# Gepeng18/Sentinel

Hardware: AMD Instinct MI355X
Metric: admission decisions/sec at 1M rules Zipf(1.1), 1/2/4/8 GPU; % HBM peak (higher is better)
Workload: dtype int64

## Files before the change

sentinel_amd/csrc/cluster.hip:

```cpp
#include "cluster.hpp"
#include "cluster_exact.hpp"
#include "cparam_exact.hpp"

#include <cstdio>
#include <cstdlib>

#include <algorithm>
#include <type_traits>

namespace sga {

namespace {

constexpr int kThreads = 256;
constexpr int kItems = 16;
constexpr int kTileElems = kThreads * kItems;

enum : uint8_t { RUN_FAST = 0, RUN_DONE = 1 };

__device__ __forceinline__ uint64_t lanemask_lt64(int lane) { return (1ULL << lane) - 1ULL; }

__device__ __forceinline__ HashEntry slot_lookup(const ClusterState &st, int64_t fid) {
    uint32_t h = (uint32_t)hash_flow_id(fid) & st.hmask;
    for (uint32_t probe = 0; probe <= st.hmask; ++probe) {
// ... 1876 lines not shown
            sc.seg_stat[kSegStat * seg] = a;
        }
        __syncthreads();
        if (active) {
            uint32_t npc = 0;
            for (int w = 0; w < wave; ++w) npc += s_np[w];
            const uint32_t pgper = (((n + kHotSeg - 1) / kHotSeg) + kPsGroups - 1) / kPsGroups;
#pragma unroll
            for (int r = 0; r < kSubRounds; ++r) {
                const uint32_t i = ubase + (uint32_t)r * 64 + lane;
                const uint32_t cd = hc[r];
                const bool hot = i < send && cd != kNoCode;
                const uint32_t hid = cd & 0xFFFu;
                const uint32_t r_seg = hot ? ((cd >> 12) & 0x1FFFu) + c[hid] : 0u;
                const bool pr = hot && (cd >> 31);
                if (i < send) sc.hcode[i] = hot ? ((cd & ~(0x1FFFu << 12)) | (r_seg << 12)) : kNoCode;
                const uint64_t em = __ballot(pr);
                if (pr) {
                    sc.pel_tile[(size_t)seg * kHotSeg + npc + (uint32_t)__popcll(em & lt)] = el_pack(hid, r_seg >> 7, 1u, r_seg & 127u, i);
                    atomicAdd(&sc.prow[(size_t)(seg / pgper) * kHot + hid], 1u);
                }
                npc += (uint32_t)__popcll(em);
            }
        }
        __syncthreads();
        const uint32_t b0 = sh.s_bmin, b1 = sh.s_bmax;
        uint32_t *pc = reinterpret_cast<uint32_t *>(&cnt[0][0]);
        for (uint32_t b = b0; b <= b1; ++b) {
            for (uint32_t k = threadIdx.x; k < nhot; k += kKeyThreads) pc[k] = 0;
            __syncthreads();
#pragma unroll
            for (int r = 0; r < kSubRounds; ++r) {
                const uint32_t cd = hc[r];
                if (ubase + (uint32_t)r * 64 + lane < send && cd != kNoCode && ((cd >> 25) & 63u) < b)
                    atomicAdd(&pc[cd & 0xFFFu], 1u);
            }
            __syncthreads();
            for (uint32_t k = threadIdx.x; k < nhot; k += kKeyThreads) sc.hpre[(size_t)b * kHot + k] = (uint16_t)pc[k];
            if (threadIdx.x == 0) atomicAdd(&sc.counters[CTL_NPRE], 1u);
            __syncthreads();
        }
    }
    {
        tmax_l = wave_max_u32(tmax_l);
        if (lane == 0) {
            sh.s_tm[wave] = tmax_l;
            sh.s_nc[wave] = nc;
        }
        __syncthreads();
        if (threadIdx.x == 0) {
            uint32_t tm = 0, a = 0, p = 0, bd = 0;
            for (int w = 0; w < kKeyWaves; ++w) {
                tm = max(tm, sh.s_tm[w]);
                a += sh.s_nc[w];
                if (nhot) {
                    p += s_np[w];
                    bd = max(bd, s_bd[w]);
                }
            }
            if (kPass == 0) {
                uint32_t *kt = sc.ktot + (seg % kKeyStripes) * kKeyStripeWords;
                if (a) atomicAdd(&kt[0], a);
                if (p) atomicAdd(&kt[1], p);
                if (bd) atomicMax(&kt[2], bd);
                if (tm) atomicMax(&kt[3], tm);
            } else if (a) {
                atomicAdd(&sc.counters[CTL_NSORT], a);
            }
        }
    }
    if (lane == 0) sc.tile_nc[sub] = active ? nc : 0u;
    if (pl) {
        __syncthreads();
        for (uint32_t k = threadIdx.x; k < (uint32_t)kPartBins; k += kKeyThreads)
            hist[(size_t)seg * kPartBins + k] = sh.phist[k];
    }
    if (d0) {
        __syncthreads();
        for (uint32_t k = threadIdx.x; k < (2u << d0); k += kKeyThreads) {
            const uint32_t t = k >> d0, d = k & dmask, tile = seg * 2 + t;
            if (tile < ntiles) hist[(size_t)d * ntiles + tile] = sh.hist0[t][d];
        }
    }
}

__global__ __launch_bounds__(256) void k_part_colscan(BatchScratch sc, uint32_t nseg) {
    const uint32_t b = blockIdx.x * 256 + threadIdx.x;
    const uint32_t t0 = blockIdx.y * kPartGroup, t1 = min(nseg, t0 + kPartGroup);
    uint32_t acc = 0;
    for (uint32_t t = t0; t < t1; t += 8) {
        uint32_t v[8];
#pragma unroll
        for (int k = 0; k < 8; ++k) v[k] = t + k < t1 ? sc.phist[(size_t)(t + k) * kPartBins + b] : 0u;
#pragma unroll
        for (int k = 0; k < 8; ++k) {
            if (t + k < t1) sc.phist[(size_t)(t + k) * kPartBins + b] = acc;
            acc += v[k];
        }
    }
    sc.pgrp[(size_t)blockIdx.y * kPartBins + b] = acc;
}

__global__ __launch_bounds__(256) void k_part_binscan(BatchScratch sc, uint32_t ngroups) {
    __shared__ uint32_t ws[4];
    __shared__ uint32_t s_last;
    const int lane = threadIdx.x & 63, wave = threadIdx.x >> 6;
    const uint32_t b = blockIdx.x * 256 + threadIdx.x;
    uint32_t acc = 0;
    for (uint32_t g = 0; g < ngroups; g += 8) {
        uint32_t v[8];
#pragma unroll
        for (int k = 0; k < 8; ++k) v[k] = g + k < ngroups ? sc.pgrp[(size_t)(g + k) * kPartBins + b] : 0u;
#pragma unroll
        for (int k = 0; k < 8; ++k) {
            if (g + k < ngroups) sc.pgrp[(size_t)(g + k) * kPartBins + b] = acc;
            acc += v[k];
        }
    }
    sc.pstart[b] = acc;
    __threadfence();
    __syncthreads();
    if (threadIdx.x == 0) s_last = atomicAdd(&sc.pstart[kPartBins + 1], 1u) == gridDim.x - 1;
    __syncthreads();
    if (!s_last) return;
    __threadfence();
    constexpr int kPer = kPartBins / 256;
    uint32_t tot[kPer], ts = 0;
#pragma unroll
    for (int k = 0; k < kPer; ++k) {
        tot[k] = __hip_atomic_load(&sc.pstart[threadIdx.x * kPer + k], __ATOMIC_RELAXED, __HIP_MEMORY_SCOPE_AGENT);
        ts += tot[k];
    }
    uint32_t x = ts;
#pragma unroll
    for (int o = 1; o < 64; o <<= 1) {
        const uint32_t y = __shfl_up(x, o, 64);
        if (lane >= o) x += y;
    }
    if (lane == 63) ws[wave] = x;
    __syncthreads();
    uint32_t pre = x - ts;
    for (int w = 0; w < wave; ++w) pre += ws[w];
#pragma unroll
    for (int k = 0; k < kPer; ++k) {
        sc.pstart[threadIdx.x * kPer + k] = pre;
        pre += tot[k];
    }
    if (threadIdx.x == 255) {
        sc.pstart[kPartBins] = pre;
        sc.pstart[kPartBins + 1] = 0;
    }
}

__global__ __launch_bounds__(kKeyThreads) void k_part_scatter(BatchScratch sc, uint32_t nseg, int lb,
                                                              uint64_t *__restrict__ out) {
    __shared__ uint32_t gb[kPartBins];
    __shared__ uint16_t wc[kKeyWaves][kPartBins];
    const uint32_t per = (nseg + 7) / 8;
    const uint32_t seg = (blockIdx.x & 7u) * per + (blockIdx.x >> 3);
    if (seg >= nseg) return;
    const uint32_t g = seg / kPartGroup;
    const int lane = threadIdx.x & 63, wave = threadIdx.x >> 6;
    const uint64_t lt = lanemask_lt64(lane);
    for (uint32_t b = threadIdx.x; b < (uint32_t)kPartBins; b += kKeyThreads) {
        gb[b] = sc.pstart[b] + sc.pgrp[(size_t)g * kPartBins + b] + sc.phist[(size_t)seg * kPartBins + b];
#pragma unroll
        for (int w = 0; w < kKeyWaves; ++w) wc[w][b] = 0;
    }
    const uint32_t sub = seg * kKeyWaves + wave;
    const uint32_t nc = sc.tile_nc[sub];
    const uint64_t *src = sc.el_tile + (size_t)sub * kSubSeg;
    uint64_t x[kSubRounds];
#pragma unroll
    for (int r = 0; r < kSubRounds; ++r) {
        const uint32_t i = (uint32_t)r * 64 + lane;
        x[r] = src[i < nc ? i : 0u];
    }
    __syncthreads();
#pragma unroll
    for (int r = 0; r < kSubRounds; ++r) {
        if ((uint32_t)r * 64 >= nc) break;
        const bool valid = (uint32_t)r * 64 + lane < nc;
        const uint32_t b = el_slot(x[r]) >> lb;
        const uint64_t peers = match_lanes(b, kPartBits, valid);
        if (valid && (peers & lt) == 0) wc[wave][b] += (uint16_t)__popcll(peers);
        __builtin_amdgcn_wave_barrier();
    }
    __syncthreads();
    for (uint32_t b = threadIdx.x; b < (uint32_t)kPartBins; b += kKeyThreads) {
        uint32_t run = 0;
#pragma unroll
        for (int w = 0; w < kKeyWaves; ++w) {
            const uint32_t c = wc[w][b];
            wc[w][b] = (uint16_t)run;
            run += c;
        }
    }
    __syncthreads();
#pragma unroll
    for (int r = 0; r < kSubRounds; ++r) {
        if ((uint32_t)r * 64 >= nc) break;
        const bool valid = (uint32_t)r * 64 + lane < nc;
        const uint32_t b = el_slot(x[r]) >> lb;
        const uint64_t peers = match_lanes(b, kPartBits, valid);
        if (valid) out[gb[b] + wc[wave][b] + (uint32_t)__popcll(peers & lt)] = x[r];
        __builtin_amdgcn_wave_barrier();
        if (valid && (peers & lt) == 0) wc[wave][b] += (uint16_t)__popcll(peers);
        __builtin_amdgcn_wave_barrier();
    }
}

template <int kPass, bool kDense, bool kNT, bool kPk>
__device__ __forceinline__ void hot_key_pass(KeyShared &sh, const ClusterState &st, const BatchScratch &sc,
                                             const ReqIn &in, int64_t ts_base, uint32_t n, uint64_t *__restrict__ out,
                                             int d0, uint32_t *__restrict__ hist, uint32_t ntiles, int pipelined) {
    const uint32_t nseg = (n + kHotSeg - 1) / kHotSeg;
    if (kPass == 0) {
        if (blockIdx.x >= nseg) {
            const uint32_t fl = hot_precheck(st, sc, in, ts_base, (blockIdx.x - nseg) * kKeyThreads + threadIdx.x,
                                             pipelined);
            if (fl) atomicOr(&sc.counters[CTL_FLAGS], fl);
            return;
        }
        hot_key<0, kDense, kNT, kPk>(sh, st, sc, in, ts_base, n, out, d0, hist, ntiles, blockIdx.x);
        return;
    }
    const uint32_t f = sc.counters[CTL_FLAGS];
    const bool rerun = (f & (kFlagRerun | kFlagState)) != 0;
    if (blockIdx.x == 0 && threadIdx.x < (uint32_t)kKeyStripes) {
        static_assert(kKeyStripes == 64, "one stripe per lane of the first wave");
        uint32_t *kt = sc.ktot + threadIdx.x * kKeyStripeWords;
        uint32_t ns = kt[0], np = kt[1], bd = kt[2], tm = kt[3];
        kt[0] = kt[1] = kt[2] = kt[3] = 0;
        ns = wave_sum_u32(ns);
        np = wave_sum_u32(np);
        bd = wave_max_u32(bd);
        tm = wave_max_u32(tm);
        if (threadIdx.x == 0) {
            atomicMax(sc.tmax_all, (unsigned long long)(ts_base + (int64_t)tm));
            if (!rerun) {
                sc.counters[CTL_NSORT] = ns;
                sc.counters[CTL_NPRIO] = np;
                sc.counters[CTL_NCOLD] = ns;
                sc.counters[CTL_BDHI] = bd;
                sc.counters[CTL_MODE] = hot_count(sc) ? 1u : 0u;
            }
        }
    }
    if (!rerun) return;
    for (uint32_t seg = blockIdx.x; seg < nseg; seg += gridDim.x) {
        hot_key<1, kDense, kNT, kPk>(sh, st, sc, in, ts_base, n, out, d0, hist, ntiles, seg);
        __syncthreads();
    }
    __threadfence();
    __syncthreads();
    if (threadIdx.x == 0) sh.s_last = atomicAdd(&sc.counters[CTL_KTICKET], 1u) == gridDim.x - 1;
    __syncthreads();
    if (!sh.s_last || threadIdx.x != 0) return;
    __threadfence();
    const uint32_t ns = ld_agent(&sc.counters[CTL_NSORT]);
    sc.counters[CTL_NCOLD] = ns;
    sc.counters[CTL_NPRIO] = 0;
    sc.counters[CTL_BDHI] = 0;
    sc.counters[CTL_MODE] = 0;
    sc.counters[CTL_KTICKET] = 0;
    if (f & kFlagState) {
        sc.counters[CTL_FLAGS] = kFlagState;
        sc.counters[CTL_BDLO] = 0;
        sc.counters[CTL_NPRE] = 0;
    }
}

template <int kPass, bool kNT = false, bool kPk = false>
__global__ __launch_bounds__(kKeyThreads) __attribute__((amdgpu_waves_per_eu(4))) void k_hot_key_dense(
    ClusterState st, BatchScratch sc, ReqIn in, int64_t ts_base, uint32_t n, uint64_t *__restrict__ out, int d0,
    uint32_t *__restrict__ hist, uint32_t ntiles, int pipelined) {
    __shared__ KeyShared sh;
    hot_key_pass<kPass, true, kNT, kPk>(sh, st, sc, in, ts_base, n, out, d0, hist, ntiles, pipelined);
}
template <int kPass, bool kPk = false>
__global__ __launch_bounds__(kKeyThreads) void k_hot_key_hash(
    ClusterState st, BatchScratch sc, ReqIn in, int64_t ts_base, uint32_t n, uint64_t *__restrict__ out, int d0,
    uint32_t *__restrict__ hist, uint32_t ntiles, int pipelined) {
    __shared__ KeyShared sh;
    hot_key_pass<kPass, false, false, kPk>(sh, st, sc, in, ts_base, n, out, d0, hist, ntiles, pipelined);
}

__global__ __launch_bounds__(kThreads) void k_hscan_group(BatchScratch sc, uint32_t nrows) {
    if (!sc.counters[CTL_MODE]) return;
    const uint32_t h = blockIdx.y * kThreads + threadIdx.x;
    if (h >= hot_count(sc)) return;
    const uint32_t r0 = blockIdx.x * kHotGroupRows;
    uint32_t s = 0;
#pragma unroll
    for (int k = 0; k < kHotGroupRows; ++k)
        if (r0 + k < nrows) s += sc.hcnt[(size_t)(r0 + k) * kHot + h];
    sc.hgsum[(size_t)blockIdx.x * kHot + h] = s;
}

__device__ __forceinline__ void psort_cols_one(const BatchScratch &sc, uint32_t h, uint32_t ngroups);
__global__ __launch_bounds__(kThreads) void k_hscan_mid(BatchScratch sc, uint32_t ngroups, uint32_t pgroups) {
    if (!sc.counters[CTL_MODE]) return;
    const uint32_t h = blockIdx.x * kThreads + threadIdx.x;
    if (pgroups) psort_cols_one(sc, h, pgroups);
    if (h >= hot_count(sc)) return;
    uint32_t acc = 0;
#pragma unroll 8
    for (uint32_t g = 0; g < ngroups; ++g) {
        const uint32_t v = sc.hgsum[(size_t)g * kHot + h];
        sc.hgsum[(size_t)g * kHot + h] = acc;
        acc += v;
    }
    sc.hot_tot[h] = acc;
}

__global__ __launch_bounds__(kThreads) void k_hscan_down(BatchScratch sc, uint32_t nrows) {
    if (!sc.counters[CTL_MODE]) return;
    const uint32_t h = blockIdx.y * kThreads + threadIdx.x;
    if (h >= hot_count(sc)) return;
    const uint32_t r0 = blockIdx.x * kHotGroupRows;
    uint32_t v[kHotGroupRows];
#pragma unroll
    for (int k = 0; k < kHotGroupRows; ++k) v[k] = r0 + k < nrows ? sc.hcnt[(size_t)(r0 + k) * kHot + h] : 0u;
    uint32_t run = sc.hgsum[(size_t)blockIdx.x * kHot + h];
#pragma unroll
    for (int k = 0; k < kHotGroupRows; ++k) {
        if (r0 + k < nrows) sc.hbase[(size_t)(r0 + k) * kHot + h] = run;
        run += v[k];
    }
}

__device__ __forceinline__ uint32_t ps_per_group(uint32_t nseg) { return (nseg + kPsGroups - 1) / kPsGroups; }

__global__ __launch_bounds__(256) void k_psort_cols(BatchScratch sc, uint32_t ngroups) {
    if (!sc.counters[CTL_MODE]) return;
    psort_cols_one(sc, blockIdx.x * 256 + threadIdx.x, ngroups);
}
__device__ __forceinline__ void psort_cols_one(const BatchScratch &sc, uint32_t h, uint32_t ngroups) {
    uint32_t acc = 0;
    constexpr int kChunk = 64;
    for (uint32_t g0 = 0; g0 < ngroups; g0 += kChunk) {
        uint32_t v[kChunk];
#pragma unroll
        for (int k = 0; k < kChunk; ++k) v[k] = g0 + k < ngroups ? sc.prow[(size_t)(g0 + k) * kHot + h] : 0u;
#pragma unroll
        for (int k = 0; k < kChunk; ++k) {
            if (g0 + k < ngroups) sc.ppre[(size_t)(g0 + k) * kHot + h] = acc;
            acc += v[k];
        }
    }
    sc.ptot[h] = acc;
}

__global__ __launch_bounds__(64) void k_psort_scatter(BatchScratch sc, uint32_t nseg, uint64_t *__restrict__ out) {
    __shared__ uint32_t base[kHot];
    const uint32_t g = blockIdx.x;
    const int lane = threadIdx.x;
    const bool mode = sc.counters[CTL_MODE] != 0;
    if (mode) {
        constexpr int kPer = kHot / 64;
        uint32_t sum = 0;
// ... 1266 lines not shown
    take(sc.phist, segs_alloc * kPartBins * 4);
    take(sc.pgrp, ((segs_alloc + kPartGroup - 1) / kPartGroup) * kPartBins * 4);
    take(sc.pstart, (kPartBins + 2) * 4);
    return off;
}

size_t batch_scratch_bytes(size_t cap, uint32_t nslots_cap) {
    BatchScratch none;
    return batch_scratch_layout(none, nullptr, cap, nslots_cap);
}

void batch_scratch_carve(BatchScratch &sc, void *base, size_t cap, uint32_t nslots_cap) {
    batch_scratch_layout(sc, (char *)base, cap, nslots_cap);
    sc.counters_clean = 0;
    sc.cap = cap;
    SGA_HIP_CHECK(hipMemset(sc.prow, 0, (size_t)kPsGroups * kHot * 4));
    SGA_HIP_CHECK(hipMemset(sc.ktot, 0, kKeyStripes * kKeyStripeWords * 4));
}

__device__ __forceinline__ uint32_t probe_mix(uint32_t x) {
    x ^= x >> 16;
    x *= 0x7feb352dU;
    x ^= x >> 15;
    x *= 0x846ca68bU;
    x ^= x >> 16;
    return x;
}
__global__ __launch_bounds__(kThreads) void k_lds_order_probe(uint32_t *bad) {
    __shared__ uint32_t cw[kThreads / 64][kHot / 2];
    const int lane = threadIdx.x & 63, w = threadIdx.x >> 6;
    const uint32_t K = 1u << (blockIdx.x % 13);
    const int mode = (blockIdx.x / 13) % 3;
    for (int k = lane; k < kHot / 2; k += 64) cw[w][k] = 0;
    __builtin_amdgcn_wave_barrier();
    const uint64_t lt = lanemask_lt64(lane);
    uint32_t nb = 0;
    for (uint32_t r = 0; r < 32; ++r) {
        const uint32_t x = probe_mix((blockIdx.x * 1315423911u) ^ (r * 2654435761u) ^ (threadIdx.x * 97u));
        uint32_t hid = x % K;
        if (mode == 1 && (x & 1u)) hid = 7 % K;
        const bool act = mode == 2 ? ((x >> 8) & 1u) : true;
        const uint32_t sh = (hid & 1u) << 4;
        const uint32_t before = (cw[w][hid >> 1] >> sh) & 0xFFFFu;
        __builtin_amdgcn_wave_barrier();
        uint64_t peers = __ballot(act);
        for (int b = 0; b < 12; ++b) {
            const bool bit = (hid >> b) & 1u;
            const uint64_t bb = __ballot(bit);
            peers &= bit ? bb : ~bb;
        }
        const uint32_t expect = before + (uint32_t)__popcll(peers & lt);
        __builtin_amdgcn_wave_barrier();
        uint32_t got = expect;
        if (act) got = rank_hot(cw[w], hid);
        __builtin_amdgcn_wave_barrier();
        if (got != expect) ++nb;
    }
    if (nb) atomicAdd(bad, nb);
}

bool lds_lane_order_ok(hipStream_t s) {
    uint32_t *d = nullptr, h = 1;
    if (hipMalloc(&d, 4) != hipSuccess) return false;
    bool ok = hipMemsetAsync(d, 0, 4, s) == hipSuccess;
    if (ok) {
        hipLaunchKernelGGL(k_lds_order_probe, dim3(13 * 3 * 64), dim3(kThreads), 0, s, d);
        ok = hipMemcpyAsync(&h, d, 4, hipMemcpyDeviceToHost, s) == hipSuccess &&
             hipStreamSynchronize(s) == hipSuccess && h == 0;
    }
    (void)hipFree(d);
    return ok;
}

void hot_reset(const ClusterState &st, BatchScratch &sc, uint32_t nslots_cap, hipStream_t s) {
    const uint32_t m = std::max(nslots_cap, st.dkey ? st.dense_n : 0u);
    hipLaunchKernelGGL(k_hot_reset, dim3(std::max<uint32_t>(1, std::min<uint32_t>((m + 255) / 256, 4096))),
                       dim3(256), 0, s, st, sc, nslots_cap);
}

static void side_stream_init(BatchScratch &sc) {
    if (sc.side) return;
    SGA_HIP_CHECK(hipStreamCreateWithFlags(&sc.side, hipStreamNonBlocking));
    const unsigned evf = hipEventDisableTiming | hipEventReleaseToDevice;
    SGA_HIP_CHECK(hipEventCreateWithFlags(&sc.ev_fork0, evf));
    SGA_HIP_CHECK(hipEventCreateWithFlags(&sc.ev_fork, evf));
    SGA_HIP_CHECK(hipEventCreateWithFlags(&sc.ev_join, evf));
    SGA_HIP_CHECK(hipEventCreateWithFlags(&sc.ev_mid, evf));
    SGA_HIP_CHECK(hipStreamCreateWithFlags(&sc.side2, hipStreamNonBlocking));
    SGA_HIP_CHECK(hipEventCreateWithFlags(&sc.ev_prio, evf));
}

static int cold_part_lb(int bits) {
    const int lb = bits - kPartBits;
    return (lb >= 5 && lb <= kPartMaxLow) ? lb : 0;
}

static int hot_key_bits(const ClusterState &st) {
    int bits = 1;
    while (((uint64_t)1 << bits) < (uint64_t)st.nslots + kHot + 2) ++bits;
    return bits;
}

static int hot_key_d0(const BatchScratch &sc, int bits) {
    const int dsort = radix64_digit_bits(bits);
    return sc.part_lb ? -sc.part_lb : (dsort <= 8 ? dsort : 0);
}

static uint32_t hot_nseg(uint32_t n) { return (n + kHotSeg - 1) / kHotSeg; }

static void hot_key_passes(const ClusterState &st, BatchScratch &sc, const ReqIn &in, int64_t ts_base, uint32_t n,
                           uint64_t *out, hipStream_t s, bool clean, bool pipelined) {
    const int bits = hot_key_bits(st);
    const uint32_t nseg = hot_nseg(n);
    if (!clean) {
        SGA_HIP_CHECK(hipMemsetAsync(sc.counters, 0, CTL_WORDS * 4, s));
        SGA_HIP_CHECK(hipMemsetAsync(sc.ktot, 0, kKeyStripes * kKeyStripeWords * 4, s));
    }
    const bool pk = in.pk != nullptr;
    auto hka = st.dense_n ? (pk ? k_hot_key_dense<0, true, true> : k_hot_key_dense<0, true, false>)
                          : (pk ? k_hot_key_hash<0, true> : k_hot_key_hash<0, false>);
    auto hkb = st.dense_n ? (pk ? k_hot_key_dense<1, false, true> : k_hot_key_dense<1, false, false>)
                          : (pk ? k_hot_key_hash<1, true> : k_hot_key_hash<1, false>);
    sc.part_lb = cold_part_lb(bits);
    const int d0 = hot_key_d0(sc, bits);
    const uint32_t ntiles_sort = (uint32_t)radix64_tiles(n);
    uint32_t *khist = sc.part_lb ? sc.phist : sc.radix.hist;
    hipLaunchKernelGGL(hka, dim3(nseg + kPreWgs), dim3(kKeyThreads), 0, s, st, sc, in, ts_base, n, out, d0, khist,
                       ntiles_sort, pipelined ? 1 : 0);
    hipLaunchKernelGGL(hkb, dim3(std::min<uint32_t>(nseg, 256)), dim3(kKeyThreads), 0, s, st, sc, in, ts_base, n, out,
                       d0, khist, ntiles_sort, 0);
}

static uint32_t ps_per_group_h(uint32_t nseg) { return std::max<uint32_t>(1, (nseg + kPsGroups - 1) / kPsGroups); }
static uint32_t ps_groups_h(uint32_t nseg) { return (nseg + ps_per_group_h(nseg) - 1) / ps_per_group_h(nseg); }

static void hot_scans(BatchScratch &sc, uint32_t nseg, uint32_t pgroups, hipStream_t hs) {
    const uint32_t ngroups = (nseg + kHotGroupRows - 1) / kHotGroupRows;
    hipLaunchKernelGGL(k_hscan_group, dim3(ngroups, kHot / kThreads), dim3(kThreads), 0, hs, sc, nseg);
    hipLaunchKernelGGL(k_hscan_mid, dim3(kHot / kThreads), dim3(kThreads), 0, hs, sc, ngroups, pgroups);
    hipLaunchKernelGGL(k_hscan_down, dim3(ngroups, kHot / kThreads), dim3(kThreads), 0, hs, sc, nseg);
}

static void prio_scatter(BatchScratch &sc, uint32_t nseg, hipStream_t ps) {
    hipLaunchKernelGGL(k_psort_scatter, dim3(kPsGroups), dim3(64), 0, ps, sc, nseg, sc.pel[0]);
    sc.pel_sorted = sc.pel[0];
}

static void cold_order(const ClusterState &st, BatchScratch &sc, uint32_t n, hipStream_t s) {
    const uint32_t nseg = hot_nseg(n);
    if (sc.part_lb) {
        const uint32_t ngroups = (nseg + kPartGroup - 1) / kPartGroup;
        hipLaunchKernelGGL(k_part_colscan, dim3(kPartBins / 256, ngroups), dim3(256), 0, s, sc, nseg);
        hipLaunchKernelGGL(k_part_binscan, dim3(kPartBins / 256), dim3(256), 0, s, sc, ngroups);
        hipLaunchKernelGGL(k_part_scatter, dim3(8 * ((nseg + 7) / 8)), dim3(kKeyThreads), 0, s, sc, nseg, sc.part_lb,
                           sc.el[0]);
        sc.el_sorted = sc.el[0];
    } else {
        const int bits = hot_key_bits(st);
        const int np = radix_sort_u64_tiled(sc.el_tile, sc.tile_nc, sc.counters + CTL_NSORT, sc.el[0], sc.el[1], n,
                                            kSlotShift, bits, sc.radix, s, hot_key_d0(sc, bits) > 0);
        sc.el_sorted = (np & 1) ? sc.el[0] : sc.el[1];
    }
}

static void hot_side(const ClusterState &st, BatchScratch &sc, int64_t ts_base, uint32_t n, uint64_t *out,
                     hipStream_t hs) {
    const uint32_t pgrid = std::max<uint32_t>(1, std::min<uint32_t>((n + kThreads - 1) / kThreads, 1024));
    hipLaunchKernelGGL(k_prio_rank, dim3(pgrid), dim3(kThreads), 0, hs, st, sc, sc.pel_sorted);
    hipLaunchKernelGGL(k_hot_flows, dim3(kHot / kH1Waves), dim3(kThreads), 0, hs, st, sc, ts_base);
    SGA_HIP_CHECK(hipEventRecord(sc.ev_mid, hs));
    hipLaunchKernelGGL(k_hot_final_g, dim3((n + kFinGSpan - 1) / kFinGSpan + kFinPrioWgsG), dim3(kFinGThreads), 0, hs,
                       st, sc, n, sc.pel_sorted, out);
    SGA_HIP_CHECK(hipEventRecord(sc.ev_join, hs));
}

static void cold_stage_and_next(const ClusterState &st, BatchScratch &sc, const ReqIn &in, int64_t ts_base,
                                uint32_t n, uint64_t *out, hipStream_t s) {
    const uint32_t hot_min = std::max<uint32_t>(sc.hot_min, 1);
    cold_stage(st, sc, sc.el_sorted, n, sc.counters + CTL_NCOLD, st.nslots, in, ts_base, 0, hot_min, out, s,
               sc.part_lb);
    if (fz_debug()) {
        unsigned long long ph[8];
        SGA_HIP_CHECK(hipMemcpyFromSymbolAsync(ph, HIP_SYMBOL(g_fz_phase), sizeof(ph), 0, hipMemcpyDeviceToHost, s));
        SGA_HIP_CHECK(hipStreamSynchronize(s));
        const unsigned long long z[8] = {0, 0, 0, 0, 0, 0, 0, 0};
        SGA_HIP_CHECK(hipMemcpyToSymbolAsync(HIP_SYMBOL(g_fz_phase), z, sizeof(z), 0, hipMemcpyHostToDevice, s));
        if (ph[7])
            fprintf(stderr, "fz phases (wall_clock64 ticks per workgroup, %llu wgs): order %.0f runs %.0f flows %.0f results %.0f\n",
                    ph[7], (double)ph[3] / ph[7], (double)ph[0] / ph[7], (double)ph[1] / ph[7], (double)ph[2] / ph[7]);
    }
    SGA_HIP_CHECK(hipStreamWaitEvent(s, sc.ev_mid, 0));
    const uint32_t sb = 64;
    hipLaunchKernelGGL(k_hot_next_a, dim3(sb), dim3(kThreads), 0, s, st, sc, hot_min);
    hipLaunchKernelGGL(k_hot_pick, dim3(sb), dim3(kThreads), 0, s, st, sc, sc.hot_min);
    SGA_HIP_CHECK(hipStreamWaitEvent(s, sc.ev_join, 0));
    hipLaunchKernelGGL(k_hot_fin, dim3(1), dim3(kFinThreads), 0, s, st, sc);
    sc.counters_clean = 1;
}

static void decide_hot_sync(const ClusterState &st, BatchScratch &sc, const ReqIn &in, int64_t ts_base, uint32_t n,
                            uint64_t *out, hipStream_t s, bool clean) {
    const uint32_t nseg = hot_nseg(n);
    hot_key_passes(st, sc, in, ts_base, n, out, s, clean, false);
    side_stream_init(sc);
    SGA_HIP_CHECK(hipEventRecord(sc.ev_fork0, s));
    SGA_HIP_CHECK(hipStreamWaitEvent(sc.side, sc.ev_fork0, 0));
    hot_scans(sc, nseg, ps_groups_h(nseg), sc.side);
    prio_scatter(sc, nseg, sc.side);
    hot_side(st, sc, ts_base, n, out, sc.side);
    cold_order(st, sc, n, s);
    cold_stage_and_next(st, sc, in, ts_base, n, out, s);
}

bool cluster_hot_eligible(const ClusterState &st, const BatchScratch &sc, uint32_t n, int simple, int nlims) {
    const bool limited = nlims > 0 && !simple;
    if (n == 0 || (n <= std::min<uint32_t>(sc.small_max, kSmall) && !limited && !radix64_lookback())) return false;
    return sc.hot_enabled && sc.hot_lane_order && !simple && !limited && !radix64_lookback() &&
           st.nslots + (uint64_t)kHot + 2 < kMaxSlots;
}

void cluster_classify_hot(const ClusterState &st, BatchScratch &sc, const int64_t *flow_id, const int32_t *acquire,
                          const uint8_t *prio, int64_t ts_base, const uint32_t *ts_off, uint32_t n, void *out,
                          hipStream_t s) {
    const bool clean = sc.counters_clean != 0;
    sc.counters_clean = 0;
    test_dispatch_reset(s);
    ReqIn in;
    in.flow = flow_id;
    in.acq = acquire;
    in.prio = prio;
    in.ts = ts_off;
    const uint32_t nseg = hot_nseg(n);
    hot_key_passes(st, sc, in, ts_base, n, (uint64_t *)out, s, clean, true);
    side_stream_init(sc);
    SGA_HIP_CHECK(hipEventRecord(sc.ev_fork0, s));
    SGA_HIP_CHECK(hipStreamWaitEvent(sc.side, sc.ev_fork0, 0));
    SGA_HIP_CHECK(hipStreamWaitEvent(sc.side2, sc.ev_fork0, 0));
    hot_scans(sc, nseg, 0u, sc.side);
    hipLaunchKernelGGL(k_psort_cols, dim3(kHot / 256), dim3(256), 0, sc.side2, sc, ps_groups_h(nseg));
    prio_scatter(sc, nseg, sc.side2);
    SGA_HIP_CHECK(hipEventRecord(sc.ev_prio, sc.side2));
    SGA_HIP_CHECK(hipStreamWaitEvent(sc.side, sc.ev_prio, 0));
    cold_order(st, sc, n, s);
    SGA_HIP_CHECK(hipEventRecord(sc.ev_fork, sc.side));
    SGA_HIP_CHECK(hipStreamWaitEvent(s, sc.ev_fork, 0));
}

void cluster_decide_hot(const ClusterState &st, BatchScratch &sc, const int32_t *acquire, const uint8_t *prio,
                        int64_t ts_base, const uint32_t *ts_off, uint32_t n, void *out, hipStream_t s) {
    ReqIn in;
    in.acq = acquire;
    in.prio = prio;
    in.ts = ts_off;
    SGA_HIP_CHECK(hipEventRecord(sc.ev_fork0, s));
    SGA_HIP_CHECK(hipStreamWaitEvent(sc.side, sc.ev_fork0, 0));
    hot_side(st, sc, ts_base, n, (uint64_t *)out, sc.side);
    cold_stage_and_next(st, sc, in, ts_base, n, (uint64_t *)out, s);
}

void cluster_decide_batch(const ClusterState &st, BatchScratch &sc, const int64_t *flow_id, const int32_t *acquire,
                          const uint8_t *prio, int64_t ts_base, const uint32_t *ts_off, uint32_t n, int simple,
                          void *out_v, hipStream_t s, const LimiterPass *lims, int nlims) {
    if (n == 0) return;
    test_dispatch_reset(s);
    ReqIn in;
    in.flow = flow_id;
    in.acq = acquire;
    in.prio = simple ? nullptr : prio;
    in.ts = ts_off;
    const bool clean = sc.counters_clean != 0;
    sc.counters_clean = 0;
    uint64_t *out = (uint64_t *)out_v;
    int bits = 1;
    while (((uint64_t)1 << bits) < (uint64_t)st.nslots + 1) ++bits;
    const uint32_t invalid_key = st.nslots;
    const bool limited = nlims > 0 && !simple;
    const int d0 = radix64_digit_bits(bits);
    const uint32_t ntiles = (n + kTileElems - 1) / kTileElems;
    static_assert(kTileElems == kRadix64Tile, "classify tiles are sort tiles");
    const bool lb = radix64_lookback() != 0;
    const int npass = (bits + d0 - 1) / d0;
    if (lb && (npass << d0) > 1024)
        throw HipError("look-back sort (SGA_RADIX_MODE=0) needs npass << digit bits <= 1024", __FILE__, __LINE__);
    if (n <= std::min<uint32_t>(sc.small_max, kSmall) && !limited && !lb) {
        uint32_t m = 64;
        while (m < n) m <<= 1;
        hipLaunchKernelGGL(k_small_sort, dim3(1), dim3(kSmallThreads), 0, s, st, flow_id, acquire, prio, ts_off, ts_base,
                           n, m, simple, invalid_key, sc.el[0], out);
        hipLaunchKernelGGL(k_cold_fused, dim3((n + kFzChunk - 1) / kFzChunk), dim3(kFzThreads), 0, s, st, sc, sc.el[0],
                           n, nullptr, invalid_key, in, ts_base, simple, 0xFFFFFFFFu, out, 0, nullptr, 0);
        return;
    }
    if (cluster_hot_eligible(st, sc, n, simple, nlims)) {
        decide_hot_sync(st, sc, in, ts_base, n, out, s, clean);
        return;
    }
    SGA_HIP_CHECK(hipMemsetAsync(sc.counters, 0, CTL_WORDS * 4, s));
    if (lb) SGA_HIP_CHECK(hipMemsetAsync(sc.radix.ghist, 0, kRadixGhistWords * sizeof(uint32_t), s));
    if (lb) SGA_HIP_CHECK(hipMemsetAsync(sc.radix.err, 0, sizeof(uint32_t), s));
    const uint64_t *el = sc.el[npass & 1];
    hipLaunchKernelGGL(k_classify, dim3(ntiles), dim3(kThreads), 0, s, st, flow_id, acquire, prio, ts_off, ts_base, n,
                       simple, invalid_key, sc.el[0], out, limited ? 0 : d0, ntiles, sc.radix.hist,
                       (lb && !limited) ? npass : 0, bits, sc.radix.ghist);
    if (!simple) apply_limiters(st.param, sc, sc.el[0], n, invalid_key, ts_base, ts_off, out, lims, nlims, s);
    const int np = radix_sort_u64(sc.el[0], sc.el[1], n, kSlotShift, bits, sc.radix, s, !limited);
    if (np != npass) throw HipError("radix pass count mismatch", __FILE__, __LINE__);
    cold_stage(st, sc, el, n, nullptr, invalid_key, in, ts_base, simple, 0xFFFFFFFFu, out, s, 0);
// ... 272 lines not shown
```

sentinel_amd/csrc/cluster.hpp:

```cpp
#pragma once
#include "../../include/sentinel_amd.h"
#include "common.hpp"
#include "radix_sort.hpp"

namespace sga {

struct SlotParam {
    double thr;
    double thr_simple;
    double isec;
    uint32_t boff;
    int32_t S;
    int32_t W;
    int32_t interval;
    int32_t active;
    int32_t ns;
};

struct SlotOcc {
    int64_t occ_pass;
    int64_t occ_preq;
    int32_t has_occ;
    int32_t pad;
};

enum : int { CEV_PASS = 0, CEV_BLOCK, CEV_PASS_REQUEST, CEV_BLOCK_REQUEST, CEV_OCCUPIED_PASS, CEV_OCCUPIED_BLOCK,
             CEV_WAITING, CEV_N };

struct alignas(16) HashEntry {
    int64_t key;
    uint32_t slot;
    uint32_t W;
};

struct ClusterState {
    const SlotParam *param;
    int64_t *rec;
    const HashEntry *htab;
    const uint32_t *dense;
    uint32_t *dkey;
    const uint32_t *wtab;
    const int64_t *slot_fid;
    uint32_t dense_n;
    uint32_t hmask;
    uint32_t nslots;
    double max_occupy_ratio;
    int32_t uni_S, uni_W, uni_iv, uni_pad;
};

constexpr uint32_t kDkHot = 0x80000000u, kDkNone = 0x7FFFFFFFu;

struct ReqIn {
    const int64_t *flow = nullptr;
    const int32_t *acq = nullptr;
    const uint8_t *prio = nullptr;
    const uint32_t *ts = nullptr;
    const uint32_t *pk = nullptr;
    __device__ __forceinline__ uint32_t ts_at(uint32_t i) const { return pk ? pk[3 * (size_t)i + 1] : ts[i]; }
    __device__ __forceinline__ int32_t acq_at(uint32_t i) const {
        return pk ? (int32_t)(pk[3 * (size_t)i + 2] & 0xFFFFu) : acq[i];
    }
    __device__ __forceinline__ bool prio_at(uint32_t i) const {
        return pk ? ((pk[3 * (size_t)i + 2] >> 16) & 1u) != 0 : (prio && prio[i]);
    }
    __device__ __forceinline__ int64_t flow_at(uint32_t i) const { return pk ? (int64_t)pk[3 * (size_t)i] : flow[i]; }
};

struct NsLimiterDev {
    int64_t start[10];
    int64_t cnt[10];
};

struct LimiterPass {
    int32_t ns;
    double qps_allowed;
    NsLimiterDev *state;
};

struct alignas(16) RunOut {
    int64_t s0;
    double thr;
    double isec;
    uint32_t f;
    uint32_t cpf;
    uint32_t cw;
    uint16_t wait;
    uint8_t mode;
    uint8_t pad;
};

struct RAgg {
    uint32_t nh, flag, cnt;
};

struct HotRun {
    int64_t s0;
    double thr;
    double isec;
    uint32_t f;
    uint32_t start;
    uint32_t n;
    uint32_t p0;
    uint32_t cpf;
    uint32_t cw;
    uint16_t wait;
    uint8_t ok;
    uint8_t pad;
    uint32_t pad2[3];
};
static_assert(sizeof(HotRun) == 64, "hot run record");

constexpr int kHot = 4096;
constexpr uint16_t kColdId = 0xFFFF;
constexpr uint32_t kNoSlot = 0xFFFFFFFFu;
constexpr int kHotCtlWords = 128;
constexpr int kHotSeg = 8192;
constexpr int kSubSeg = 1024;
constexpr int kHotBuckets = 64;
constexpr int kHotGroupRows = 16;
constexpr int kHotCand = 1 << 16;
constexpr int kSegStat = 4;
constexpr int kKeyStripes = 64;
constexpr int kKeyStripeWords = 32;
constexpr int kPartBits = 11;
constexpr int kPartBins = 1 << kPartBits;
constexpr int kPartGroup = 64;
constexpr int kPartMaxLow = 10;

enum : int {
    CTL_NVALID = 0, CTL_NRUNS = 1, CTL_NFLOWS = 2, CTL_LIMITED = 4, CTL_LIMRUNS = 5, CTL_DEFERRED = 6,
    CTL_FLAGS = 16,
    CTL_NPRIO = 19,
    CTL_NSORT = 20,
    CTL_NCOLD = 21,
    CTL_NPRE = 22,
    CTL_BDLO = 23,
    CTL_BDHI = 24,
    CTL_MODE = 25,
    CTL_HOTERR = 26,
    CTL_KTICKET = 27,
    CTL_WORDS = 64
};
enum : uint32_t {
    kFlagUnsorted = 1,
    kFlagMixed = 2,
    kFlagBucket = 4,
    kFlagHotKey = 8,
    kFlagRerun = 15,
    kFlagState = 16
};

struct WConst {
    uint32_t W, r0;
    double inv;
};

struct BatchScratch {
    uint64_t *el[2];
    uint32_t *run_start, *run_slot, *run_idx0, *run_cp, *run_p0;
    int32_t *run_acq;
    uint8_t *run_bd;
    uint32_t *flow_first_run;
    uint32_t *plist;
    RunOut *run_out;
    RAgg *wave_carry;
    void *tile_agg;
    void *tile_carry;
    uint32_t *tile_valid;
    uint32_t *counters;
    uint32_t *counters_last;
    int counters_clean = 0;
    uint32_t *lim_partial;
    RadixScratch radix;
    size_t cap = 0;
    uint16_t *hot_of;
    uint32_t *hot_slot;
    uint32_t *hot_next;
    uint32_t *hot_ctl;
    uint64_t *el_tile;
    uint32_t *tile_nc;
    uint64_t *pel_tile;
    uint32_t *prow;
    uint32_t *ppre;
    uint32_t *ptot;
    uint64_t *pel[2];
    uint32_t *hcode;
    uint16_t *hcnt;
    uint32_t *hbase;
    uint32_t *hgsum;
    uint16_t *hpre;
    uint32_t *hbnd;
    HotRun *hrun;
    uint32_t *prank;
    uint32_t *plo, *phi;
    uint32_t *hot_tot;
    uint32_t *seg_stat;
    uint32_t *ktot;
    unsigned long long *tmax_all;
    const uint64_t *el_sorted = nullptr, *pel_sorted = nullptr;
    uint32_t *hot_cand;
    uint32_t *phist, *pgrp, *pstart;
    int part_lb = 0;
    int hot_enabled = 1;
    uint32_t small_max = 4096;
    int hot_lane_order = 0;
    uint32_t hot_min = 64;
    hipStream_t side = nullptr;
    hipEvent_t ev_fork = nullptr, ev_join = nullptr, ev_fork0 = nullptr, ev_mid = nullptr;
    hipStream_t side2 = nullptr;
    hipEvent_t ev_prio = nullptr;
};

bool lds_lane_order_ok(hipStream_t stream);

void hot_reset(const ClusterState &st, BatchScratch &b, uint32_t nslots_cap, hipStream_t stream);
void batch_scratch_release(BatchScratch &b);

constexpr size_t kMaxBatch = (size_t)1 << 26;
constexpr uint32_t kMaxSlots = (1u << 24) - 2;

size_t batch_scratch_bytes(size_t cap, uint32_t nslots_cap);
void batch_scratch_carve(BatchScratch &b, void *base, size_t cap, uint32_t nslots_cap);

void cluster_decide_batch(const ClusterState &st, BatchScratch &sc, const int64_t *flow_id, const int32_t *acquire,
                          const uint8_t *prio, int64_t ts_base, const uint32_t *ts_off, uint32_t n, int simple,
                          void *out , hipStream_t stream, const LimiterPass *lims = nullptr,
                          int nlims = 0);
void cluster_decide_batch_packed(const ClusterState &st, BatchScratch &sc, const uint32_t *pk, int64_t ts_base,
                                 uint32_t n, void *out, hipStream_t stream, const LimiterPass *lims = nullptr,
                                 int nlims = 0);

bool cluster_hot_eligible(const ClusterState &st, const BatchScratch &sc, uint32_t n, int simple, int nlims);
void cluster_classify_hot(const ClusterState &st, BatchScratch &sc, const int64_t *flow_id, const int32_t *acquire,
                          const uint8_t *prio, int64_t ts_base, const uint32_t *ts_off, uint32_t n, void *out,
                          hipStream_t stream);
void cluster_decide_hot(const ClusterState &st, BatchScratch &sc, const int32_t *acquire, const uint8_t *prio,
                        int64_t ts_base, const uint32_t *ts_off, uint32_t n, void *out, hipStream_t stream);

struct PRuleParam {
    double count;
    double isec;
    uint32_t boff;
    int32_t S, W, interval;
    int32_t active, ns, threshold_type;
    uint32_t hot_off, n_hot;
    uint32_t cap;
};

struct PLruRec {
    uint64_t kidx;
    uint64_t stamp;
};
constexpr uint64_t kPNoQueue = ~0ull;
constexpr uint64_t kPLruBuilding = ~0ull;

struct CParamState {
    const PRuleParam *param;
    int64_t *rstart;
    int64_t *tmax;
    uint8_t *coupled;
    const HashEntry *htab;
    uint32_t hmask, nslots;
    const int64_t *hot_v;
    const int32_t *hot_c;
    const int32_t *ns_connected;
    int64_t *vtab;
    uint32_t vmask;
    uint64_t *ktab;
    uint32_t kmask;
    uint32_t *koff;
    uint32_t *kslot;
    int64_t *kval;
    int64_t *krec;
    uint64_t krec_cap;
    uint32_t *ctl;
    uint32_t *nkeys;
    uint64_t *pq;
    uint32_t *psize;
    PLruRec *lpool;
// ... 46 lines not shown
```

Measured before the change: 24.43 billion.

## Scatter two partition segments per workgroup with atomic counting and vectorized bin init

```diff
diff --git a/sentinel_amd/csrc/cluster.hip b/sentinel_amd/csrc/cluster.hip
--- a/sentinel_amd/csrc/cluster.hip
+++ b/sentinel_amd/csrc/cluster.hip
@@ -2052,39 +2052,92 @@
     }
 }
 
+__device__ __forceinline__ void part_list(const BatchScratch &sc, uint32_t sub0, uint32_t nsub, int lane,
+                                          uint32_t (&cum)[kPartSpan + 1]) {
+    const uint32_t mine = lane < kPartSpan && sub0 + (uint32_t)lane < nsub ? sc.tile_nc[sub0 + lane] : 0u;
+    cum[0] = 0;
+#pragma unroll
+    for (int j = 0; j < kPartSpan; ++j) cum[j + 1] = cum[j] + (uint32_t)__builtin_amdgcn_readlane((int)mine, j);
+}
+
+__device__ __forceinline__ void part_load(const BatchScratch &sc, uint32_t sub0, const uint32_t (&cum)[kPartSpan + 1],
+                                          uint32_t c0, int lane, uint64_t (&x)[kSubRounds]) {
+#pragma unroll
+    for (int r = 0; r < kSubRounds; ++r) {
+        const uint32_t i = c0 + (uint32_t)r * 64 + lane;
+        uint32_t at = i;
+#pragma unroll
+        for (int j = 1; j < kPartSpan; ++j)
+            if (i >= cum[j]) at = (uint32_t)j * kSubSeg + (i - cum[j]);
+        x[r] = i < cum[kPartSpan] ? sc.el_tile[(size_t)sub0 * kSubSeg + at] : 0ull;
+    }
+}
+
+__device__ __forceinline__ void part_count_add(uint16_t *wcw, uint32_t b) {
+    (void)__hip_atomic_fetch_add(reinterpret_cast<uint32_t *>(wcw) + (b >> 1), 1u << ((b & 1u) * 16), __ATOMIC_RELAXED,
+                                 __HIP_MEMORY_SCOPE_WORKGROUP);
+}
+__device__ __forceinline__ void part_count_add(uint32_t *wcw, uint32_t b) {
+    (void)__hip_atomic_fetch_add(wcw + b, 1u, __ATOMIC_RELAXED, __HIP_MEMORY_SCOPE_WORKGROUP);
+}
+
+template <bool kPlace, typename Cnt>
+__device__ __forceinline__ void part_rounds(const uint64_t (&x)[kSubRounds], uint32_t c0, uint32_t total,
+                                            const uint32_t *gb, Cnt *wcw, int lb, uint64_t *__restrict__ out,
+                                            int lane) {
+    const uint64_t lt = lanemask_lt64(lane);
+#pragma unroll
+    for (int r = 0; r < kSubRounds; ++r) {
+        if (c0 + (uint32_t)r * 64 >= total) break;
+        const bool valid = c0 + (uint32_t)r * 64 + lane < total;
+        const uint32_t b = el_slot(x[r]) >> lb;
+        if (!kPlace) {
+            if (valid) part_count_add(wcw, b);
+            continue;
+        }
+        const uint64_t peers = match_lanes(b, kPartBits, valid);
+        if (valid) out[gb[b] + wcw[b] + (uint32_t)__popcll(peers & lt)] = x[r];
+        __builtin_amdgcn_wave_barrier();
+        if (valid && (peers & lt) == 0) wcw[b] += (Cnt)__popcll(peers);
+        __builtin_amdgcn_wave_barrier();
+    }
+}
+
 __global__ __launch_bounds__(kKeyThreads) void k_part_scatter(BatchScratch sc, uint32_t nseg, int lb,
                                                               uint64_t *__restrict__ out) {
-    __shared__ uint32_t gb[kPartBins];
-    __shared__ uint16_t wc[kKeyWaves][kPartBins];
-    const uint32_t per = (nseg + 7) / 8;
-    const uint32_t seg = (blockIdx.x & 7u) * per + (blockIdx.x >> 3);
-    if (seg >= nseg) return;
-    const uint32_t g = seg / kPartGroup;
+    static_assert(kPartBins == 4 * kKeyThreads, "four consecutive bins per thread");
+    using Cnt = std::conditional_t<(kPartSpan * kHotSeg <= 65535), uint16_t, uint32_t>;
+    __shared__ __attribute__((aligned(16))) uint32_t gb[kPartBins];
+    __shared__ __attribute__((aligned(16))) Cnt wc[kKeyWaves][kPartBins];
+    const uint32_t nspan = (nseg + kPartSpan - 1) / kPartSpan;
+    const uint32_t per = (nspan + 7) / 8;
+    const uint32_t span = (blockIdx.x & 7u) * per + (blockIdx.x >> 3);
+    if (span >= nspan) return;
+    const uint32_t seg0 = span * kPartSpan;
+    const uint32_t g = seg0 / kPartGroup;
     const int lane = threadIdx.x & 63, wave = threadIdx.x >> 6;
-    const uint64_t lt = lanemask_lt64(lane);
-    for (uint32_t b = threadIdx.x; b < (uint32_t)kPartBins; b += kKeyThreads) {
-        gb[b] = sc.pstart[b] + sc.pgrp[(size_t)g * kPartBins + b] + sc.phist[(size_t)seg * kPartBins + b];
-#pragma unroll
-        for (int w = 0; w < kKeyWaves; ++w) wc[w][b] = 0;
-    }
-    const uint32_t sub = seg * kKeyWaves + wave;
-    const uint32_t nc = sc.tile_nc[sub];
-    const uint64_t *src = sc.el_tile + (size_t)sub * kSubSeg;
+    const uint32_t sub0 = seg0 * kKeyWaves + (uint32_t)wave * kPartSpan;
+    uint32_t cum[kPartSpan + 1];
+    part_list(sc, sub0, nseg * kKeyWaves, lane, cum);
+    const uint32_t total = cum[kPartSpan];
     uint64_t x[kSubRounds];
-#pragma unroll
-    for (int r = 0; r < kSubRounds; ++r) {
-        const uint32_t i = (uint32_t)r * 64 + lane;
-        x[r] = src[i < nc ? i : 0u];
+    part_load(sc, sub0, cum, 0u, lane, x);
+    const uint32_t b4 = threadIdx.x * 4;
+    const uint4 st4 = *reinterpret_cast<const uint4 *>(sc.pstart + b4);
+    const uint4 gp = *reinterpret_cast<const uint4 *>(sc.pgrp + (size_t)g * kPartBins + b4);
+    const uint4 row = *reinterpret_cast<const uint4 *>(sc.phist + (size_t)seg0 * kPartBins + b4);
+    *reinterpret_cast<uint4 *>(&gb[b4]) =
+        make_uint4(st4.x + gp.x + row.x, st4.y + gp.y + row.y, st4.z + gp.z + row.z, st4.w + gp.w + row.w);
+    {
+        uint32_t *z = reinterpret_cast<uint32_t *>(&wc[0][0]);
+        for (uint32_t i = threadIdx.x; i < (uint32_t)(sizeof(wc) / 4); i += kKeyThreads) z[i] = 0;
     }
     __syncthreads();
-#pragma unroll
-    for (int r = 0; r < kSubRounds; ++r) {
-        if ((uint32_t)r * 64 >= nc) break;
-        const bool valid = (uint32_t)r * 64 + lane < nc;
-        const uint32_t b = el_slot(x[r]) >> lb;
-        const uint64_t peers = match_lanes(b, kPartBits, valid);
-        if (valid && (peers & lt) == 0) wc[wave][b] += (uint16_t)__popcll(peers);
-        __builtin_amdgcn_wave_barrier();
+    for (uint32_t c0 = 0;;) {
+        part_rounds<false>(x, c0, total, gb, wc[wave], lb, out, lane);
+        c0 += kSubSeg;
+        if (c0 >= total) break;
+        part_load(sc, sub0, cum, c0, lane, x);
     }
     __syncthreads();
     for (uint32_t b = threadIdx.x; b < (uint32_t)kPartBins; b += kKeyThreads) {
@@ -2092,21 +2145,14 @@
 #pragma unroll
         for (int w = 0; w < kKeyWaves; ++w) {
             const uint32_t c = wc[w][b];
-            wc[w][b] = (uint16_t)run;
+            wc[w][b] = (Cnt)run;
             run += c;
         }
     }
     __syncthreads();
-#pragma unroll
-    for (int r = 0; r < kSubRounds; ++r) {
-        if ((uint32_t)r * 64 >= nc) break;
-        const bool valid = (uint32_t)r * 64 + lane < nc;
-        const uint32_t b = el_slot(x[r]) >> lb;
-        const uint64_t peers = match_lanes(b, kPartBits, valid);
-        if (valid) out[gb[b] + wc[wave][b] + (uint32_t)__popcll(peers & lt)] = x[r];
-        __builtin_amdgcn_wave_barrier();
-        if (valid && (peers & lt) == 0) wc[wave][b] += (uint16_t)__popcll(peers);
-        __builtin_amdgcn_wave_barrier();
+    for (uint32_t c0 = 0; c0 < total; c0 += kSubSeg) {
+        if (total > (uint32_t)kSubSeg) part_load(sc, sub0, cum, c0, lane, x);
+        part_rounds<true>(x, c0, total, gb, wc[wave], lb, out, lane);
     }
 }
 
@@ -3679,7 +3725,8 @@
         const uint32_t ngroups = (nseg + kPartGroup - 1) / kPartGroup;
         hipLaunchKernelGGL(k_part_colscan, dim3(kPartBins / 256, ngroups), dim3(256), 0, s, sc, nseg);
         hipLaunchKernelGGL(k_part_binscan, dim3(kPartBins / 256), dim3(256), 0, s, sc, ngroups);
-        hipLaunchKernelGGL(k_part_scatter, dim3(8 * ((nseg + 7) / 8)), dim3(kKeyThreads), 0, s, sc, nseg, sc.part_lb,
+        const uint32_t nspan = (nseg + kPartSpan - 1) / kPartSpan;
+        hipLaunchKernelGGL(k_part_scatter, dim3(8 * ((nspan + 7) / 8)), dim3(kKeyThreads), 0, s, sc, nseg, sc.part_lb,
                            sc.el[0]);
         sc.el_sorted = sc.el[0];
     } else {
diff --git a/sentinel_amd/csrc/cluster.hpp b/sentinel_amd/csrc/cluster.hpp
--- a/sentinel_amd/csrc/cluster.hpp
+++ b/sentinel_amd/csrc/cluster.hpp
@@ -125,6 +125,8 @@
 constexpr int kPartBits = 11;
 constexpr int kPartBins = 1 << kPartBits;
 constexpr int kPartGroup = 64;
+constexpr int kPartSpan = 2;
+static_assert(kPartGroup % kPartSpan == 0, "a scatter span lies inside one group of the column scan");
 constexpr int kPartMaxLow = 10;
 
 enum : int {
```

Measured after the change: 24.83 billion, median of 6. 1.6% higher.
